# vkit-dev/vkit-ocr-model-adaptive-scaling

Measured on AMD Instinct MI355X. Metric: images/sec fwd+bwd @1024x1024 bf16 (train step: rough+precise passes, losses, backward, clip, AdamW), higher is better.
Workload: dtype bf16

## Files before the change

include/vkas.h:

```cpp
#ifndef VKAS_H
#define VKAS_H

#include <stddef.h>
#include <stdint.h>

#ifdef __cplusplus
extern "C" {
#endif

#define VKAS_F32 0
#define VKAS_BF16 1
#define VKAS_F16 2

#define VKAS_OK 0
#define VKAS_E_ARG (-1)
#define VKAS_E_LAUNCH (-2)

#define VKAS_EPI_NONE 0
#define VKAS_EPI_GELU 1
#define VKAS_EPI_SCALE_RES 2
#define VKAS_EPI_DGELU 3
#define VKAS_EPI_ADD 4
#define VKAS_EPI_PATCH 5
#define VKAS_EPI_HEAD 6
// ... 77 lines not shown
                       const float* colscale, const float* rowscale, int rows_per_image, void* h, long ldh, void* z,
                       long ldz, void* out, long ldo, long M, int C, int dtype, void* stream);
int vkas_mlp_chain_ln_fwd(const void* y, long ldy, const float* ln_gamma, const float* ln_beta, void* yn, long ldyn,
                          float* stats, const void* img, const float* b2, const void* x, long ldx, const float* colscale,
                          const float* rowscale, int rows_per_image, void* h, long ldh, void* z, long ldz, void* out,
                          long ldo, long M, int C, int dtype, void* stream);
int vkas_mlp_chain_bwd(const void* dz, long lddz, const void* img_t, const void* h, long ldh, void* dh, long lddh,
                       void* dyn, long lddyn, long M, int C, int dtype, void* stream);
int vkas_conv_gemm_tile(int wgrad, long M, int Np, int K);
int vkas_conv_gemm_kernel_id(int wgrad, const vkas_conv_geom* g, int Np, long lddy, int head_width);
typedef struct vkas_gemm_switches {
  int nt_tile, tn_tile;
  int nt_ring;
  int nt_noslab, nt_nobuf, tn_nobuf, tn_noslab, tn_no96;
} vkas_gemm_switches;
typedef struct vkas_gemm_plan_info {
  int kernel_id, family, bn, ring, buf, head, pw, nobias, xg;
  long grid_m, grid_n, tiles, splits, rows, a_bytes, b_bytes;
  unsigned grid;
  char name[44];
} vkas_gemm_plan_info;
int vkas_conv_gemm_plan(int wgrad, const vkas_conv_geom* g, int Np, long lddy, int head_width, int flags, int has_gb,
                        const vkas_gemm_switches* sw, vkas_gemm_plan_info* out);
int vkas_colsum(const void* y, long ld, long M, int Np, float* out, int accumulate, float* ws, size_t ws_bytes,
                int dtype, void* stream);
size_t vkas_colsum_ws_bytes(long M, int Np);

int vkas_dwconv7x7_fwd(const void* x, long ldx, const float* w, const float* bias, const void* addend, long ldadd,
                       void* y, long ldy, int B, int H, int W, int Cp, int dtype, void* stream);
int vkas_dwconv7x7_wgrad(const void* x, long ldx, const void* dy, long lddy, float* gw, float* gb, float* ws,
                         size_t ws_bytes, int B, int H, int W, int Cp, int dtype, void* stream);
size_t vkas_dwconv7x7_wgrad_ws_bytes(int B, int H, int W, int Cp);

int vkas_layernorm_fwd(const void* x, long ldx, const float* gamma, const float* beta, void* y, long ldy,
                       float* stats, long M, int C, int Cp, int act_gelu, int dtype, void* stream);
int vkas_layernorm_bwd(const void* x, long ldx, const float* gamma, const float* beta, const float* stats,
                       const void* dy, long lddy, void* dx, long lddx, float* dgamma, float* dbeta, float* ws,
                       size_t ws_bytes, long M, int C, int Cp, int act_gelu, int dtype, void* stream);
size_t vkas_layernorm_bwd_ws_bytes(long M, int Cp);

int vkas_pack_head_params(const float* gamma, const float* beta, const float* wproj, const float* bproj, int C, int oc,
                          int pw, float* out, void* stream);
int vkas_head_tail_fwd(const void* z, long ldz, const vkas_head_desc* hd, long M, int dtype, void* stream);
int vkas_head_tail_bwd(const void* z, long ldz, const vkas_head_desc* hd, const float* const* dproj, void* dz, long lddz,
                       float* dparams, float* ws, size_t ws_bytes, long M, int dtype, void* stream);
size_t vkas_head_tail_bwd_ws_bytes(long M, int pw);
// ... 165 lines not shown
```

vkit_ocr_model_adaptive_scaling_amd/_lib.py:

```python
import ctypes
import os
from ctypes import POINTER, Structure, c_char, c_char_p, c_double, c_float, c_int, c_int64, c_long, c_longlong, c_size_t, c_uint, c_void_p

_HERE = os.path.dirname(os.path.abspath(__file__))
LIB_PATH = os.environ.get('VKAS_LIB_PATH') or os.path.join(_HERE, 'libvkas.so')

F32, BF16, F16 = 0, 1, 2
EPI_NONE, EPI_GELU, EPI_SCALE_RES, EPI_DGELU, EPI_ADD, EPI_PATCH, EPI_HEAD = range(7)
LOSS_FOCAL, LOSS_DICE, LOSS_L1, LOSS_SMOOTH_L1, LOSS_L2 = range(5)
LOSS_WAHR = 5
PRECISE_LOSS_EX_SUMS = 16


class ConvGeom(Structure):
    _fields_ = [('B', c_int), ('Hin', c_int), ('Win', c_int), ('Hout', c_int), ('Wout', c_int), ('Cp', c_int),
                ('ldx', c_int), ('KH', c_int), ('KW', c_int), ('stride', c_int), ('pad', c_int)]


class HeadDesc(Structure):
    _fields_ = [('n_heads', c_int), ('pw', c_int), ('n0', c_int * 4), ('np', c_int * 4), ('c', c_int * 4),
                ('oc', c_int * 4), ('params', c_void_p), ('stats', c_void_p), ('proj', c_void_p)]


class Epilogue(Structure):
    _fields_ = [('mode', c_int), ('bias', c_void_p), ('out', c_void_p), ('ldo', c_long), ('out2', c_void_p),
                ('ldo2', c_long), ('aux', c_void_p), ('ldaux', c_long), ('colscale', c_void_p),
                ('rowscale', c_void_p), ('rows_per_image', c_int), ('patch', c_int), ('patch_Hs', c_int),
                ('patch_Ws', c_int), ('patch_Cp', c_int), ('head', HeadDesc)]


class GemmSwitches(Structure):
    _fields_ = [('nt_tile', c_int), ('tn_tile', c_int), ('nt_ring', c_int), ('nt_noslab', c_int), ('nt_nobuf', c_int),
                ('tn_nobuf', c_int), ('tn_noslab', c_int), ('tn_no96', c_int)]

    def __init__(self, nt_ring=-1, **kw):
        super().__init__(nt_ring=nt_ring, **kw)


class GemmPlanInfo(Structure):
    _fields_ = [(n, c_int) for n in ('kernel_id', 'family', 'bn', 'ring', 'buf', 'head', 'pw', 'nobias', 'xg')] + \
               [(n, c_long) for n in ('grid_m', 'grid_n', 'tiles', 'splits', 'rows', 'a_bytes', 'b_bytes')] + \
               [('grid', c_uint), ('name', c_char * 44)]


class PackDesc(Structure):
    _fields_ = [('w', c_void_p), ('out', c_void_p), ('total', c_long), ('kind', c_int), ('N', c_int), ('C', c_int),
                ('KH', c_int), ('KW', c_int), ('Np', c_int), ('Cp', c_int), ('mode', c_int), ('n_off', c_int),
                ('Nt', c_int), ('dtype', c_int)]


class RoughLossCfg(Structure):
    _fields_ = [('focal_factor', c_float), ('dice_factor', c_float), ('l1_factor', c_float), ('score_min', c_float),
                ('height_min', c_float), ('focal_alpha', c_float), ('focal_gamma', c_float), ('out_scale', c_float)]


class PreciseLossCfg(Structure):
    _fields_ = [('pos_l2', c_float), ('neg_l2', c_float), ('offset_l1', c_float), ('reg_l1', c_float),
                ('angle_ce', c_float), ('dist_l1', c_float), ('loss_factor', c_float), ('smooth_beta', c_float),
                ('out_scale', c_float)]


class PreciseLossExtraCfg(Structure):
    _fields_ = [('mask_focal', c_float), ('prob_l1', c_float), ('prob_wahr', c_float), ('prob_l1_beta', c_float),
                ('wahr_gamma', c_float), ('focal_alpha', c_float), ('focal_gamma', c_float)]

# ... 31 lines not shown
    'vkas_nchw_f32_to_nhwc': (c_int, [_P, _P, c_long, c_int, c_int, c_int, c_int, c_int, c_int, _P]),
    'vkas_conv_gemm_fwd': (c_int, [_P, POINTER(ConvGeom), _P, c_int, POINTER(Epilogue), c_int, _P]),
    'vkas_conv_gemm_wgrad': (c_int, [_P, POINTER(ConvGeom), _P, c_long, c_int, _P, _P, c_int, _P]),
    'vkas_conv_gemm_wgrad_ordered': (c_int, [_P, POINTER(ConvGeom), _P, c_long, c_int, _P, c_int, _P]),
    'vkas_conv_gemm_wgrad_gelu': (c_int, [_P, POINTER(ConvGeom), _P, c_long, c_int, _P, _P, c_int, _P]),
    'vkas_upconv5_fold_elems': (c_size_t, [c_int, c_int, c_int, c_int]),
    'vkas_upconv5_fold': (c_int, [_P, _P, c_int, c_int, c_int, c_int, c_int, c_int, c_int, _P]),
    'vkas_upconv5_fwd': (c_int, [_P, POINTER(ConvGeom), c_int, _P, c_int, _P, _P, c_long, c_int, _P]),
    'vkas_upconv5_dgrad': (c_int, [_P, c_long, POINTER(ConvGeom), c_int, _P, c_int, _P, c_long, c_int, _P]),
    'vkas_upconv5_wgrad_ws_bytes': (c_size_t, [c_int, c_int, c_int, c_int]),
    'vkas_upconv5_wgrad': (c_int, [_P, POINTER(ConvGeom), c_int, _P, c_long, c_int, _P, c_size_t, _P, _P, c_int, _P]),
    'vkas_upconv5_unfold_wgrad': (c_int, [_P, _P, c_int, c_int, c_int, c_int, c_int, c_int, _P]),
    'vkas_mlp_chain_image_elems': (c_size_t, [c_int]),
    'vkas_mlp_chain_pack': (c_int, [_P, _P, _P, c_int, c_int, _P, c_int, _P]),
    'vkas_mlp_chain_fwd': (c_int, [_P, c_long, _P, _P, _P, c_long, _P, _P, c_int, _P, c_long, _P, c_long, _P, c_long,
                                   c_long, c_int, c_int, _P]),
    'vkas_mlp_chain_ln_fwd': (c_int, [_P, c_long, _P, _P, _P, c_long, _P, _P, _P, _P, c_long, _P, _P, c_int, _P, c_long, _P,
                                      c_long, _P, c_long, c_long, c_int, c_int, _P]),
    'vkas_mlp_chain_bwd': (c_int, [_P, c_long, _P, _P, c_long, _P, c_long, _P, c_long, c_long, c_int, c_int, _P]),
    'vkas_conv_gemm_tile': (c_int, [c_int, c_long, c_int, c_int]),
    'vkas_conv_gemm_kernel_id': (c_int, [c_int, POINTER(ConvGeom), c_int, c_long, c_int]),
    'vkas_conv_gemm_plan': (c_int, [c_int, POINTER(ConvGeom), c_int, c_long, c_int, c_int, c_int, POINTER(GemmSwitches),
                                    POINTER(GemmPlanInfo)]),
    'vkas_colsum': (c_int, [_P, c_long, c_long, c_int, _P, c_int, _P, c_size_t, c_int, _P]),
    'vkas_colsum_ws_bytes': (c_size_t, [c_long, c_int]),
    'vkas_dwconv7x7_fwd': (c_int, [_P, c_long, _P, _P, _P, c_long, _P, c_long, c_int, c_int, c_int, c_int, c_int, _P]),
    'vkas_dwconv7x7_wgrad': (c_int, [_P, c_long, _P, c_long, _P, _P, _P, c_size_t, c_int, c_int, c_int, c_int, c_int, _P]),
    'vkas_dwconv7x7_wgrad_ws_bytes': (c_size_t, [c_int, c_int, c_int, c_int]),
    'vkas_layernorm_fwd': (c_int, [_P, c_long, _P, _P, _P, c_long, _P, c_long, c_int, c_int, c_int, c_int, _P]),
    'vkas_layernorm_bwd': (c_int, [_P, c_long, _P, _P, _P, _P, c_long, _P, c_long, _P, _P, _P, c_size_t, c_long, c_int,
                                   c_int, c_int, c_int, _P]),
    'vkas_layernorm_bwd_ws_bytes': (c_size_t, [c_long, c_int]),
    'vkas_pack_head_params': (c_int, [_P, _P, _P, _P, c_int, c_int, c_int, _P, _P]),
    'vkas_head_tail_fwd': (c_int, [_P, c_long, _P, c_long, c_int, _P]),
    'vkas_head_tail_bwd': (c_int, [_P, c_long, POINTER(HeadDesc), POINTER(c_void_p), _P, c_long, _P, _P, c_size_t, c_long, c_int, _P]),
    'vkas_head_tail_bwd_ws_bytes': (c_size_t, [c_long, c_int]),
    'vkas_scale_res_bwd': (c_int, [_P, c_long, _P, c_long, _P, _P, c_int, _P, c_long, _P, _P, _P, c_size_t, c_long,
                                   c_int, c_int, _P]),
    'vkas_scale_res_bwd_ws_bytes': (c_size_t, [c_long, c_int]),
    'vkas_resize_fwd': (c_int, [_P, c_long, _P, c_long, c_int, c_int, c_int, c_int, c_int, c_int, c_int, c_int, c_int, _P]),
    'vkas_resize_bwd': (c_int, [_P, c_long, _P, c_long, c_int, c_int, c_int, c_int, c_int, c_int, c_int, c_int, c_int, _P]),
    'vkas_resize_bwd_ws_bytes': (c_size_t, [c_int, c_int, c_int, c_int, c_int, c_int]),
    'vkas_resize_bwd_ws': (c_int, [_P, c_long, _P, c_long, _P, c_size_t, c_int, c_int, c_int, c_int, c_int, c_int, c_int, c_int,
                                   c_int, _P]),
    'vkas_upconv_adj': (c_int, [_P, c_long, _P, c_int, c_int, c_int, c_int, c_int, _P]),
    'vkas_upconv_adj_colsum_ws_bytes': (c_size_t, [c_int, c_int, c_int, c_int]),
# ... 67 lines not shown
```

vkit_ocr_model_adaptive_scaling_amd/csrc/gemm_api.hip:

```cpp
#include <stdlib.h>
#include <string.h>

#include "gemm_parts.h"
#include "gemm_plan.h"

int vkas_gemm_nt_simple(const void*, const vkas_conv_geom*, const void*, int, const vkas_epilogue*, int, hipStream_t);
int vkas_gemm_tn_simple(const void*, const vkas_conv_geom*, const void*, long, int, float*, float*, int, int, hipStream_t);
int vkas_gemm_nt_mfma_bf16(const void*, const vkas_conv_geom*, const void*, int, const vkas_epilogue*, hipStream_t);
int vkas_gemm_tn_mfma_bf16(const void*, const vkas_conv_geom*, const void*, long, int, float*, float*, int, hipStream_t);
int vkas_gemm_nt_mfma_f16(const void*, const vkas_conv_geom*, const void*, int, const vkas_epilogue*, hipStream_t);
int vkas_gemm_tn_mfma_f16(const void*, const vkas_conv_geom*, const void*, long, int, float*, float*, int, hipStream_t);

static thread_local char g_err[512] = "";

void vkas_set_error(const char* fmt, ...) {
  va_list ap;
  va_start(ap, fmt);
  vsnprintf(g_err, sizeof(g_err), fmt, ap);
  va_end(ap);
}

extern "C" const char* vkas_last_error(void) { return g_err; }
extern "C" int vkas_abi_version(void) { return 1; }

static bool force_simple() {
  static int v = -1;
  if (v < 0) {
// ... 71 lines not shown

extern "C" int vkas_conv_gemm_plan(int wgrad, const vkas_conv_geom* g, int Np, long lddy, int head_width, int flags, int has_gb,
                                   const vkas_gemm_switches* sw, vkas_gemm_plan_info* out) {
  VKAS_CHECK(g && out, "vkas_conv_gemm_plan: null argument");
  vkas_gemm_plan_info o = {};
  if (!sw && force_simple()) {
    snprintf(o.name, sizeof(o.name), wgrad ? "gemm_tn_simple" : "gemm_nt_simple");
  } else if (wgrad) {
    const vkas_tn_plan p = vkas_plan_tn(*g, Np, lddy, flags, has_gb != 0, sw ? *sw : *vkas_gemm_env_switches());
    o = {vkas_tn_kernel_id(p), p.family, p.tile, 0, p.buf, 0, p.pw, p.nobias, p.xg, 0, 0, p.tiles, p.splits, p.rows, p.x_bytes, p.dy_bytes, p.grid, ""};
    const char* t = p.tile == 128 ? "2,2,4" : (p.tile == 192 ? "2,4,6" : (p.tile == 224 ? "2,4,7" : "4,2,6"));
    if (p.family == VKAS_TN_SLAB) snprintf(o.name, sizeof(o.name), "conv3x3_wgrad_slab_kernel<%d>", p.tile / 16);
    else snprintf(o.name, sizeof(o.name), "gemm_tn_mfma_kernel<%s,4>", t);
  } else {
    const vkas_nt_plan p = vkas_plan_nt(*g, Np, head_width, sw ? *sw : *vkas_gemm_env_switches());
    const long tiles = p.grid_m * p.grid_n;
    o = {vkas_nt_kernel_id(p), p.family, p.bn, p.ring, p.buf, p.head, 0, 0, 0, p.grid_m, p.grid_n, tiles, 1, 0, p.a_bytes, p.b_bytes, (unsigned)tiles, ""};
    if (p.family == VKAS_NT_SLAB) snprintf(o.name, sizeof(o.name), "conv3x3_slab_mfma_kernel<%d,%d>", p.bn / 32, (int)p.head);
    else if (p.family == VKAS_NT_RING) snprintf(o.name, sizeof(o.name), "gemm_nt_ring_kernel<%d>", p.ring);
    else snprintf(o.name, sizeof(o.name), "gemm_nt_mfma_kernel<%s,4,%d>", p.family == VKAS_NT_REG128 ? "2,2" : "4,2", p.bn / 32);
  }
  *out = o;
  return VKAS_OK;
}

extern "C" int vkas_conv_gemm_tile(int wgrad, long M, int Np, int K) {
  if (force_simple()) return 0;
  const vkas_gemm_switches& sw = *vkas_gemm_env_switches();
  return wgrad ? vkas_tn_tile_rule(M, Np, K, sw) : vkas_nt_tile_rule(M, Np, sw);
}

extern "C" int vkas_conv_gemm_kernel_id(int wgrad, const vkas_conv_geom* g, int Np, long lddy, int head_width) {
  vkas_gemm_plan_info o;
  return g && vkas_conv_gemm_plan(wgrad, g, Np, lddy, head_width, 0, 0, nullptr, &o) == VKAS_OK ? o.kernel_id : 0;
}

static int conv_gemm_wgrad(const char* who, const void* x, const vkas_conv_geom* g, const void* dy, long lddy, int Np,
                           float* gw, float* gb, int x_gelu, int dtype, void* stream) {
  int rc = vkas_check_geom(who, x, g, Np);
  if (rc) return rc;
  VKAS_CHECK(dy && vkas_aligned16(dy) && lddy >= Np && lddy % 8 == 0, "%s: bad dy (lddy=%ld)", who, lddy);
  VKAS_CHECK(gw, "%s: null gw", who);
  if (dtype == VKAS_BF16 && !force_simple())
    return vkas_gemm_tn_mfma_bf16(x, g, dy, lddy, Np, gw, gb, x_gelu, vkas_stream(stream));
  if (dtype == VKAS_F16 && !force_simple())
    return vkas_gemm_tn_mfma_f16(x, g, dy, lddy, Np, gw, gb, x_gelu, vkas_stream(stream));
// ... 183 lines not shown
```

vkit_ocr_model_adaptive_scaling_amd/csrc/gemm_mfma.hip:

```cpp
#include <stdlib.h>

#include <type_traits>

#include "gemm_parts.h"
#include "gemm_plan.h"

#ifdef VKAS_MFMA_F16
typedef f16_t elem_t;
typedef f16x8 elem8;
typedef f16x4 elem4;
#define VKAS_MFMA16(a, b, c, x, y, z) __builtin_amdgcn_mfma_f32_16x16x32_f16(a, b, c, x, y, z)
#define VKAS_MFMA_FN(name) name##_f16
#else
typedef bf16_t elem_t;
typedef bf16x8 elem8;
typedef bf16x4 elem4;
#define VKAS_MFMA16(a, b, c, x, y, z) __builtin_amdgcn_mfma_f32_16x16x32_bf16(a, b, c, x, y, z)
#define VKAS_MFMA_FN(name) name##_bf16
#endif

namespace {

constexpr int BK = 64;

#ifndef VKAS_ABL
#define VKAS_ABL 0
#endif
constexpr int ABL = VKAS_ABL;
// ... 80 lines not shown
      load8(hp + (2 + qq) * pw + c0, w);
#pragma unroll
      for (int c = 0; c < 8; ++c) pr[qq] = fmaf(a[c], w[c], pr[qq]);
    }
  }
#pragma unroll
  for (int qq = 0; qq < 4; ++qq) {
    if (qq >= oc) break;
    pr[qq] = group_sum<LPR>(pr[qq]);
  }
  if (j == 0 && m < M) {
    const float4 bp = *reinterpret_cast<const float4*>(hp + 6 * pw);
    float* po = e.head.proj + ((long)head * M + m) * 8;
    *reinterpret_cast<float4*>(po) = make_float4(pr[0] + bp.x, pr[1] + bp.y, pr[2] + bp.z, pr[3] + bp.w);
    *reinterpret_cast<float4*>(po + 4) = make_float4(0.f, 0.f, 0.f, 0.f);
    if (e.head.stats) {
      float* st = e.head.stats + ((long)head * M + m) * 2;
      st[0] = mean;
      st[1] = rstd;
    }
  }
}

template <int WM, int WN, int TM, int TN, bool HEAD>
__device__ __forceinline__ void nt_epilogue(f32x4 (&acc)[TM][TN], float* stage, const vkas_epilogue& e, int tile_n,
                                            long m0, long M, int n0, int n_end, int tid) {
  constexpr int NTHR = WM * WN * 64;
  constexpr int BM = WM * TM * 16, BN = WN * TN * 16;
  constexpr int VPR = BN / 8;
  const int lane = tid & 63;
  const int wave = tid >> 6;
  const int wm = wave / WN, wn = wave % WN;
  if constexpr (!HEAD) {
    constexpr int PB = BN * 2 + 16;
    static_assert(BM * PB <= 2 * (BM + BN) * BK * 2, "single-pass staging must fit the tile buffers");
    char* st = reinterpret_cast<char*>(stage);
#pragma unroll
    for (int j = 0; j < TN; ++j) {
      const int cl = wn * TN * 16 + j * 16 + (lane >> 4) * 4;
      float4 b = make_float4(0.f, 0.f, 0.f, 0.f);
      if (e.bias && n0 + cl < n_end) b = *reinterpret_cast<const float4*>(e.bias + n0 + cl);
#pragma unroll
      for (int i = 0; i < TM; ++i) {
        const int row = wm * TM * 16 + i * 16 + (lane & 15);
        float v[4] = {acc[i][j][0] + b.x, acc[i][j][1] + b.y, acc[i][j][2] + b.z, acc[i][j][3] + b.w};
        store4(reinterpret_cast<elem_t*>(st + row * PB) + cl, v);
      }
    }
    constexpr int NIT = (BM * VPR + NTHR - 1) / NTHR;
    const bool pre = e.aux != nullptr && (e.mode == VKAS_EPI_SCALE_RES || e.mode == VKAS_EPI_DGELU || e.mode == VKAS_EPI_ADD);
    Raw8<elem_t> auxr[NIT];
    if (pre) {
#pragma unroll
      for (int it = 0; it < NIT; ++it) {
        const int t = tid + it * NTHR;
        const int row = t / VPR, c8 = t - row * VPR;
        const long m = m0 + row;
        const int n = n0 + c8 * 8;
        auxr[it].zero();
        if (t < BM * VPR && m < M && n < n_end) auxr[it].load(reinterpret_cast<const elem_t*>(e.aux) + m * e.ldaux + n);
      }
    }
    __syncthreads();
    vkas_epilogue e2 = e;
    e2.bias = nullptr;
    if (pre) {
#pragma unroll
      for (int it = 0; it < NIT; ++it) {
        const int t = tid + it * NTHR;
        const int row = t / VPR, c8 = t - row * VPR;
        const long m = m0 + row;
        const int n = n0 + c8 * 8;
        if (t < BM * VPR && m < M && n < n_end) {
          float v[8];
          load8(reinterpret_cast<const elem_t*>(st + row * PB) + c8 * 8, v);
          epi_store8<elem_t>(e2, m, n, v, &auxr[it]);
        }
      }
    } else {
#pragma unroll 2
      for (int t = tid; t < BM * VPR; t += NTHR) {
        const int row = t / VPR, c8 = t - row * VPR;
        const long m = m0 + row;
        const int n = n0 + c8 * 8;
        if (m < M && n < n_end) {
          float v[8];
          load8(reinterpret_cast<const elem_t*>(st + row * PB) + c8 * 8, v);
          epi_store8<elem_t>(e2, m, n, v);
        }
      }
    }
  } else {
    constexpr int EP = BN + 4;
    constexpr int ER = TM * 16;
    float* hp_s = stage + ER * EP;
    {
      const int pw = e.head.pw, PSZ = 6 * pw + 8;
      const float* src = e.head.params + (long)tile_n * PSZ;
      for (int i = tid; i < PSZ; i += NTHR) hp_s[i] = src[i];
    }
#pragma unroll 1
    for (int pass = 0; pass < WM; ++pass) {
      if (wm == pass) {
#pragma unroll
        for (int i = 0; i < TM; ++i)
#pragma unroll
          for (int j = 0; j < TN; ++j)
            *reinterpret_cast<f32x4*>(stage + (i * 16 + (lane & 15)) * EP + wn * TN * 16 + j * 16 + (lane >> 4) * 4) =
                acc[i][j];
      }
      __syncthreads();
      if constexpr ((ABL & 256) == 0)
        head_tail_rows<NTHR, ER, EP, VPR>(e, tile_n, stage, hp_s, m0 + (long)pass * ER, M, n0, n_end - n0, tid);
      __syncthreads();
    }
  }
}

template <int WM, int WN, int TM, int TN, bool BUF, bool HEAD>
__global__ __launch_bounds__(WM* WN * 64) void gemm_nt_mfma_kernel(const elem_t* __restrict__ x, vkas_conv_geom g,
                                                                  const elem_t* __restrict__ Bw, int Np, long M, int K,
                                                                  vkas_epilogue e, unsigned a_bytes, unsigned b_bytes) {
  constexpr int NTHR = WM * WN * 64;
  constexpr int BM = WM * TM * 16, BN = WN * TN * 16;
  constexpr int RSTEP = NTHR / 8;
  constexpr int ACH = BM / RSTEP;
  constexpr int BCH = (BN + RSTEP - 1) / RSTEP;
  static_assert(BM % RSTEP == 0, "A tile must be covered by whole staging passes");
  __shared__ __attribute__((aligned(16))) elem_t lds[2 * (BM + BN) * BK];
  const int tid = threadIdx.x;
  const int lane = tid & 63;
  const int wave = tid >> 6;
  const int wm = wave / WN, wn = wave % WN;
  constexpr bool head_mode = HEAD;
  const unsigned ntile_n = head_mode ? (unsigned)e.head.n_heads : (unsigned)((Np + BN - 1) / BN);
  VKAS_TR(0);
// ... 525 lines not shown
              acc[i][j] = VKAS_MFMA16(fb[h][j], fa[h][i], acc[i][j], 0, 0, 0);
        __builtin_amdgcn_s_setprio(0);
      }
      if (grp == 0) retire();
      if constexpr ((ABL & 4) == 0) __builtin_amdgcn_s_barrier();
      asm volatile("" ::: "memory");
    };
    sub(std::integral_constant<int, 0>{});
    sub(std::integral_constant<int, 1>{});
    sub(std::integral_constant<int, 2>{});
    ky = ky1;
    cb = cb1;
  };
  int s = 0;
  for (; s + 1 < NS; s += 2) {
    step(std::integral_constant<int, 0>{}, s);
    step(std::integral_constant<int, 1>{}, s + 1);
  }
  if (s < NS) step(std::integral_constant<int, 0>{}, s);
  if (grp == 0) __builtin_amdgcn_s_barrier();
  nt_epilogue<WM, WN, TM, TN, HEAD>(acc, (float*)lds, e, tile_n, m0, M, n0, n_end, tid);
}

template <int TN, bool HEAD>
__global__ __launch_bounds__(512) void conv3x3_slab_mfma_kernel(const elem_t* __restrict__ x, vkas_conv_geom g,
                                                                const elem_t* __restrict__ Bw, int Np, long M, int K,
                                                                vkas_epilogue e, unsigned a_bytes, unsigned b_bytes) {
  constexpr int BN = 32 * TN;
  __shared__ __attribute__((aligned(1024))) elem_t lds[2 * SLAB + 3 * BN * BK];
  const unsigned ntile_n = HEAD ? (unsigned)e.head.n_heads : (unsigned)((Np + BN - 1) / BN);
  const unsigned total = gridDim.x;
  const unsigned xcd = blockIdx.x & 7u, slot8 = blockIdx.x >> 3;
  const unsigned q8 = total >> 3, r8 = total & 7u;
  unsigned tile = (xcd < r8 ? xcd * (q8 + 1) : r8 * (q8 + 1) + (xcd - r8) * q8) + slot8;
  if constexpr (HEAD && (EXPS & 4) != 0) {
    if (ntile_n == 4 && (total & 31u) == 0) {
      const unsigned mt = total >> 2;
      const unsigned m_tile = (xcd & 3u) * (mt >> 2) + (slot8 >> 1);
      tile = m_tile * 4u + (xcd >> 2) * 2u + (slot8 & 1u);
    }
  }
  if constexpr (HEAD && TN == 7) {
    if (e.head.np[tile % ntile_n] <= 192) {
      conv3x3_slab_body<6, true, BN>(x, g, Bw, Np, M, K, e, a_bytes, b_bytes, (lds_elem*)lds, tile, ntile_n);
      return;
    }
  }
  conv3x3_slab_body<TN, HEAD, BN>(x, g, Bw, Np, M, K, e, a_bytes, b_bytes, (lds_elem*)lds, tile, ntile_n);
}

constexpr int TN_ROWS = VKAS_TN_ROWS;

__device__ __forceinline__ float dot2_ones(unsigned pair, float acc) {
#ifdef VKAS_MFMA_F16
  typedef _Float16 h2 __attribute__((ext_vector_type(2)));
  const h2 one = {(_Float16)1.0f, (_Float16)1.0f};
  return __builtin_amdgcn_fdot2(__builtin_bit_cast(h2, pair), one, acc, false);
#else
  typedef __bf16 b2 __attribute__((ext_vector_type(2)));
  const b2 one = {(__bf16)1.0f, (__bf16)1.0f};
  return __builtin_amdgcn_fdot2_f32_bf16(__builtin_bit_cast(b2, pair), one, acc, false);
#endif
}

template <int LD>
__device__ __forceinline__ elem8 tr_frag(const elem_t* tile, int mbase, int colbase, int lane) {
  const int g4 = lane >> 4, idx = lane & 15, q = idx >> 2, p = idx & 3;
  const elem_t* a0 = tile + (mbase + 4 * g4 + q) * LD + colbase + 4 * p;
  const elem_t* a1 = a0 + 16 * LD;
  const s16x4 lo = __builtin_amdgcn_ds_read_tr16_b64_v4i16((s16x4 __attribute__((address_space(3)))*)(a0));
  const s16x4 hi = __builtin_amdgcn_ds_read_tr16_b64_v4i16((s16x4 __attribute__((address_space(3)))*)(a1));
// ... 531 lines not shown
#if defined(VKAS_TRACE) && !defined(VKAS_MFMA_F16)
extern "C" int vkas_trace_read(void* dst, size_t bytes) {
  return (int)hipMemcpyFromSymbol(dst, HIP_SYMBOL(vkas_trace_buf), bytes, 0, hipMemcpyDeviceToHost);
}
#endif

static constexpr int nt_case(int family, int v, bool buf, bool head) { return ((family * 8 + v) * 2 + buf) * 2 + head; }
static constexpr int tn_case(int family, int tile, bool xg, int form) { return ((family * 512 + tile) * 2 + xg) * 4 + form; }

int VKAS_MFMA_FN(vkas_gemm_nt_mfma)(const void* x, const vkas_conv_geom* g, const void* Bw, int Np, const vkas_epilogue* e,
                           hipStream_t st) {
  const long M = (long)g->B * g->Hout * g->Wout;
  const int K = g->KH * g->KW * g->Cp;
  if (M == 0) return VKAS_OK;
  const bool head = e->mode == VKAS_EPI_HEAD;
  int wmax = 0;
  for (int h = 0; head && h < e->head.n_heads; ++h) wmax = e->head.np[h] > wmax ? e->head.np[h] : wmax;
  const vkas_nt_plan p = vkas_plan_nt(*g, Np, wmax, *vkas_gemm_env_switches());
  const dim3 grid((unsigned)(p.grid_m * (head ? e->head.n_heads : p.grid_n)));
  const unsigned ab = p.buf ? (unsigned)p.a_bytes : 0u, bb = p.buf ? (unsigned)p.b_bytes : 0u;
#define VKAS_GO(THREADS, ...) \
  __VA_ARGS__<<<grid, THREADS, 0, st>>>((const elem_t*)x, *g, (const elem_t*)Bw, Np, M, K, *e, ab, bb); \
  break;
#define VKAS_TILE(TNV)                                                                                      \
  case nt_case(VKAS_NT_TILE256, TNV, true, true): VKAS_GO(512, gemm_nt_mfma_kernel<4, 2, 4, TNV, true, true>)    \
  case nt_case(VKAS_NT_TILE256, TNV, false, true): VKAS_GO(512, gemm_nt_mfma_kernel<4, 2, 4, TNV, false, true>)  \
  case nt_case(VKAS_NT_TILE256, TNV, true, false): VKAS_GO(512, gemm_nt_mfma_kernel<4, 2, 4, TNV, true, false>)  \
  case nt_case(VKAS_NT_TILE256, TNV, false, false): VKAS_GO(512, gemm_nt_mfma_kernel<4, 2, 4, TNV, false, false>) \
  case nt_case(VKAS_NT_SLAB, TNV, true, true): VKAS_GO(512, conv3x3_slab_mfma_kernel<TNV, true>)                \
  case nt_case(VKAS_NT_SLAB, TNV, true, false): VKAS_GO(512, conv3x3_slab_mfma_kernel<TNV, false>)
  switch (nt_case(p.family, p.family == VKAS_NT_RING ? p.ring : p.bn / 32, p.buf, p.head)) {
    VKAS_TILE(4) VKAS_TILE(6) VKAS_TILE(7)
    case nt_case(VKAS_NT_REG128, 4, true, false): VKAS_GO(256, gemm_nt_mfma_kernel<2, 2, 4, 4, true, false>)
    case nt_case(VKAS_NT_REG128, 4, false, false): VKAS_GO(256, gemm_nt_mfma_kernel<2, 2, 4, 4, false, false>)
    case nt_case(VKAS_NT_RING, 2, true, false): VKAS_GO(512, gemm_nt_ring_kernel<2>)
    case nt_case(VKAS_NT_RING, 3, true, false): VKAS_GO(512, gemm_nt_ring_kernel<3>)
    case nt_case(VKAS_NT_RING, 4, true, false): VKAS_GO(512, gemm_nt_ring_kernel<4>)
    default: VKAS_CHECK(false, "gemm_nt_mfma: no kernel for family %d, N extent %d", (int)p.family, p.bn);
  }
#undef VKAS_TILE
#undef VKAS_GO
  static const char* const who[] = {"gemm_nt_mfma", "gemm_nt_ring", "gemm_nt_mfma", "conv3x3_slab_mfma"};
  VKAS_LAUNCH_CHECK(who[p.family]);
  return VKAS_OK;
}

int VKAS_MFMA_FN(vkas_gemm_tn_mfma)(const void* x, const vkas_conv_geom* g, const void* dy, long lddy, int Np, float* gw,
                           float* gb, int flags, hipStream_t st) {
  const long M = (long)g->B * g->Hout * g->Wout;
  const int K = g->KH * g->KW * g->Cp;
  if (M == 0) return VKAS_OK;
  const vkas_tn_plan p = vkas_plan_tn(*g, Np, lddy, flags, gb != nullptr, *vkas_gemm_env_switches());
  const unsigned xb = p.buf ? (unsigned)p.x_bytes : 0u, db = p.buf ? (unsigned)p.dy_bytes : 0u;
#define VKAS_GO(THREADS, ROWS, ...) \
  __VA_ARGS__<<<p.grid, THREADS, 0, st>>>((const elem_t*)x, *g, (const elem_t*)dy, lddy, Np, M, K, ROWS, gw, gb, xb, db); \
  break;
#define VKAS_TILE(WN, WK, TNn, XG)                                                                                             \
  case tn_case(VKAS_TN_GENERIC, WN * TNn * 16, XG, 0): VKAS_GO(WN * WK * 64, p.rows, gemm_tn_mfma_kernel<WN, WK, TNn, 4, false, XG>) \
  case tn_case(VKAS_TN_GENERIC, WN * TNn * 16, XG, 1): VKAS_GO(WN * WK * 64, p.rows, gemm_tn_mfma_kernel<WN, WK, TNn, 4, true, XG>)  \
  case tn_case(VKAS_TN_GENERIC, WN * TNn * 16, XG, 2): VKAS_GO(WN * WK * 64, p.rows, gemm_tn_mfma_kernel<WN, WK, TNn, 4, true, XG, true>)
  switch (tn_case(p.family, p.tile, p.xg, p.nobias ? 3 : (p.pw ? 2 : p.buf))) {
    VKAS_TILE(2, 2, 4, false) VKAS_TILE(2, 4, 6, false) VKAS_TILE(2, 4, 7, false) VKAS_TILE(4, 2, 6, false)
    VKAS_TILE(2, 2, 4, true) VKAS_TILE(2, 4, 6, true) VKAS_TILE(2, 4, 7, true) VKAS_TILE(4, 2, 6, true)
    case tn_case(VKAS_TN_GENERIC, 192, false, 3): VKAS_GO(512, p.rows, gemm_tn_mfma_kernel<2, 4, 6, 4, true, false, true, true>)
// ... 12 lines not shown
```

vkit_ocr_model_adaptive_scaling_amd/csrc/gemm_plan.h:

```cpp
#pragma once
#include "../../include/vkas.h"

constexpr int VKAS_TN_ROWS = 64;

enum vkas_nt_family { VKAS_NT_REG128, VKAS_NT_RING, VKAS_NT_TILE256, VKAS_NT_SLAB };
enum vkas_tn_family { VKAS_TN_GENERIC, VKAS_TN_SLAB };

struct vkas_nt_plan {
  vkas_nt_family family;
  int bn;
  int ring;
  bool buf, head;
  long a_bytes, b_bytes;
  long grid_m, grid_n;
};

struct vkas_tn_plan {
  vkas_tn_family family;
  int tile;
  bool buf, pw, nobias, xg;
  long splits, rows;
  long tiles;
  unsigned grid;
  long x_bytes, dy_bytes;
};

const vkas_gemm_switches* vkas_gemm_env_switches();

inline long vkas_span_bytes(long rows, long ld, long width) { return ((rows - 1) * ld + width) * 2; }
inline bool vkas_fits_buffer(long bytes) { return bytes < 0xFFFFFFF0L; }

int vkas_nt_tile_rule(long M, int Np, const vkas_gemm_switches& sw);
int vkas_tn_tile_rule(long M, int Np, int K, const vkas_gemm_switches& sw);

vkas_nt_plan vkas_plan_nt(const vkas_conv_geom& g, int Np, int head_width, const vkas_gemm_switches& sw);
vkas_tn_plan vkas_plan_tn(const vkas_conv_geom& g, int Np, long lddy, int flags, bool has_gb, const vkas_gemm_switches& sw);

inline int vkas_nt_kernel_id(const vkas_nt_plan& p) {
  return p.family == VKAS_NT_SLAB ? 1000 + p.bn / 32 : (p.family == VKAS_NT_RING ? 10 + p.ring : (p.family == VKAS_NT_REG128 ? 1 : p.bn));
}
inline int vkas_tn_kernel_id(const vkas_tn_plan& p) { return p.family == VKAS_TN_SLAB ? 2000 + p.tile / 16 : p.tile; }
```

vkit_ocr_model_adaptive_scaling_amd/csrc/gemm_plan.hip:

```cpp
#include "gemm_plan.h"

#include <stdlib.h>

#include <initializer_list>

static long cdiv(long a, long b) { return (a + b - 1) / b; }
static long padded(long n, long t) { return cdiv(n, t) * t; }

const vkas_gemm_switches* vkas_gemm_env_switches() {
  static const vkas_gemm_switches sw = [] {
    const auto num = [](const char* name, int unset) { return getenv(name) ? atoi(getenv(name)) : unset; };
    const auto set = [](const char* name) { return (int)(getenv(name) != nullptr); };
    return vkas_gemm_switches{num("VKAS_NT_TILE", 0), num("VKAS_TN_TILE", 0), num("VKAS_NT_RING", -1), set("VKAS_NT_NOSLAB"),
                              set("VKAS_NT_NOBUF"),   set("VKAS_TN_NOBUF"),   set("VKAS_TN_NOSLAB"),   set("VKAS_TN_NO96")};
  }();
  return &sw;
}

static bool row_aligned_3x3(const vkas_conv_geom& g, int wmod) {
  return g.KH == 3 && g.KW == 3 && g.stride == 1 && g.pad == 1 && g.Hout == g.Hin && g.Wout == g.Win && g.Win % wmod == 0;
}

int vkas_nt_tile_rule(long M, int Np, const vkas_gemm_switches& sw) {
  const int f = sw.nt_tile;
  if (f == 1 || f == 128 || f == 192 || f == 224) return f;
  if (M < 16384) return 1;
  int bn = 224;
  for (int c : {192, 128})
    if (padded(Np, c) < padded(Np, bn)) bn = c;
  return bn;
}

int vkas_tn_tile_rule(long M, int Np, int K, const vkas_gemm_switches& sw) {
  const int f = sw.tn_tile;
  if (f == 128 || f == 192 || f == 224 || f == 384) return f;
  int bn = 128;
  if (M >= 16384 && K >= 192) {
    for (int c : {192, 224})
      if (padded(Np, c) <= padded(Np, bn)) bn = c;
// ... 82 lines not shown
```

Before: 280.9.

## Add 2D band tiling form for 3x3 slab conv with row-piece slot ring

Adds a band variant of the 3x3 slab conv kernel in which each 256-row M tile covers a 4-row by 64-pixel image patch rather than a run of 256 pixels along one image row. Input rows are streamed as pieces into an 8-slot LDS ring and reused across the ky taps of neighbouring wave rows, with per-step waitcnt scheduling. The epilogue maps rows to the band layout. The form is on by default when the image height is divisible by 4, and it adds considerable complexity in the scheduling and in the vmcnt bookkeeping.

```diff
diff --git a/include/vkas.h b/include/vkas.h
--- a/include/vkas.h
+++ b/include/vkas.h
@@ -123,6 +123,14 @@
 } vkas_gemm_plan_info;
 int vkas_conv_gemm_plan(int wgrad, const vkas_conv_geom* g, int Np, long lddy, int head_width, int flags, int has_gb,
                         const vkas_gemm_switches* sw, vkas_gemm_plan_info* out);
+int vkas_conv_slab_form(int form);
+typedef struct vkas_slab_band_step {
+  int cb, ky, kx, fill_cb, fill_piece, fill_slot, read_slot[4], requests, wait;
+} vkas_slab_band_step;
+typedef struct vkas_slab_band_info {
+  int slots, slot_rows, slot_bytes, region_bytes, prologue_pieces, requests_per_piece;
+} vkas_slab_band_info;
+int vkas_conv_slab_band_schedule(int ncb, vkas_slab_band_info* info, vkas_slab_band_step* out, int cap);
 int vkas_colsum(const void* y, long ld, long M, int Np, float* out, int accumulate, float* ws, size_t ws_bytes,
                 int dtype, void* stream);
 size_t vkas_colsum_ws_bytes(long M, int Np);
diff --git a/vkit_ocr_model_adaptive_scaling_amd/_lib.py b/vkit_ocr_model_adaptive_scaling_amd/_lib.py
--- a/vkit_ocr_model_adaptive_scaling_amd/_lib.py
+++ b/vkit_ocr_model_adaptive_scaling_amd/_lib.py
@@ -41,6 +41,15 @@
     _fields_ = [(n, c_int) for n in ('kernel_id', 'family', 'bn', 'ring', 'buf', 'head', 'pw', 'nobias', 'xg')] + \
                [(n, c_long) for n in ('grid_m', 'grid_n', 'tiles', 'splits', 'rows', 'a_bytes', 'b_bytes')] + \
                [('grid', c_uint), ('name', c_char * 44)]
+
+
+class SlabBandStep(Structure):
+    _fields_ = [(n, c_int) for n in ('cb', 'ky', 'kx', 'fill_cb', 'fill_piece', 'fill_slot')] + \
+               [('read_slot', c_int * 4), ('requests', c_int), ('wait', c_int)]
+
+
+class SlabBandInfo(Structure):
+    _fields_ = [(n, c_int) for n in ('slots', 'slot_rows', 'slot_bytes', 'region_bytes', 'prologue_pieces', 'requests_per_piece')]
 
 
 class PackDesc(Structure):
@@ -118,6 +127,8 @@
     'vkas_conv_gemm_kernel_id': (c_int, [c_int, POINTER(ConvGeom), c_int, c_long, c_int]),
     'vkas_conv_gemm_plan': (c_int, [c_int, POINTER(ConvGeom), c_int, c_long, c_int, c_int, c_int, POINTER(GemmSwitches),
                                     POINTER(GemmPlanInfo)]),
+    'vkas_conv_slab_form': (c_int, [c_int]),
+    'vkas_conv_slab_band_schedule': (c_int, [c_int, POINTER(SlabBandInfo), POINTER(SlabBandStep), c_int]),
     'vkas_colsum': (c_int, [_P, c_long, c_long, c_int, _P, c_int, _P, c_size_t, c_int, _P]),
     'vkas_colsum_ws_bytes': (c_size_t, [c_long, c_int]),
     'vkas_dwconv7x7_fwd': (c_int, [_P, c_long, _P, _P, _P, c_long, _P, c_long, c_int, c_int, c_int, c_int, c_int, _P]),
diff --git a/vkit_ocr_model_adaptive_scaling_amd/csrc/gemm_api.hip b/vkit_ocr_model_adaptive_scaling_amd/csrc/gemm_api.hip
--- a/vkit_ocr_model_adaptive_scaling_amd/csrc/gemm_api.hip
+++ b/vkit_ocr_model_adaptive_scaling_amd/csrc/gemm_api.hip
@@ -3,6 +3,7 @@
 
 #include "gemm_parts.h"
 #include "gemm_plan.h"
+#include "slab_band_plan.h"
 
 int vkas_gemm_nt_simple(const void*, const vkas_conv_geom*, const void*, int, const vkas_epilogue*, int, hipStream_t);
 int vkas_gemm_tn_simple(const void*, const vkas_conv_geom*, const void*, long, int, float*, float*, int, int, hipStream_t);
@@ -120,6 +121,30 @@
   }
   *out = o;
   return VKAS_OK;
+}
+
+extern "C" int vkas_conv_slab_band_schedule(int ncb, vkas_slab_band_info* info, vkas_slab_band_step* out, int cap) {
+  if (ncb < 1 || cap < 0 || (cap > 0 && !out)) return -1;
+  if (info)
+    *info = {VKAS_BAND_SLOTS, VKAS_BAND_SLOT_ROWS, VKAS_BAND_SLOT_ROWS * 128, 2 * 264 * 128, VKAS_BAND_PROLOGUE, VKAS_BAND_REQ};
+  int n = 0, sb = 0;
+  for (int cb = 0; cb < ncb; ++cb, sb = vkas_band_slot(1, sb)) {
+    const bool nxt = cb + 1 < ncb;
+    for (int ky = 0; ky < 3; ++ky)
+      for (int kx = 0; kx < 3; ++kx, ++n) {
+        if (n >= cap) continue;
+        const bool more = ky < 2 || nxt;
+        const int piece = vkas_band_issue_piece(ky, kx);
+        vkas_slab_band_step s = {cb, ky, kx, -1, -1, -1, {0, 0, 0, 0}, 0, 0};
+        if (piece >= VKAS_BAND_PIECES && nxt) s.fill_cb = cb + 1, s.fill_piece = piece - VKAS_BAND_PIECES;
+        else if (piece >= 0 && piece < VKAS_BAND_PIECES) s.fill_cb = cb, s.fill_piece = piece;
+        if (s.fill_piece >= 0) s.fill_slot = (sb + piece) & (VKAS_BAND_SLOTS - 1), s.requests = VKAS_BAND_REQ;
+        for (int wm = 0; wm < 4; ++wm) s.read_slot[wm] = (sb + vkas_band_read_piece(ky, wm)) & (VKAS_BAND_SLOTS - 1);
+        s.wait = more ? vkas_band_requests(ky, kx, nxt) : -1;
+        out[n] = s;
+      }
+  }
+  return n;
 }
 
 extern "C" int vkas_conv_gemm_tile(int wgrad, long M, int Np, int K) {
diff --git a/vkit_ocr_model_adaptive_scaling_amd/csrc/gemm_mfma.hip b/vkit_ocr_model_adaptive_scaling_amd/csrc/gemm_mfma.hip
--- a/vkit_ocr_model_adaptive_scaling_amd/csrc/gemm_mfma.hip
+++ b/vkit_ocr_model_adaptive_scaling_amd/csrc/gemm_mfma.hip
@@ -4,6 +4,7 @@
 
 #include "gemm_parts.h"
 #include "gemm_plan.h"
+#include "slab_band_plan.h"
 
 #ifdef VKAS_MFMA_F16
 typedef f16_t elem_t;
@@ -130,9 +131,11 @@
   }
 }
 
-template <int WM, int WN, int TM, int TN, bool HEAD>
+template <int WM, int WN, int TM, int TN, bool HEAD, bool BAND = false>
 __device__ __forceinline__ void nt_epilogue(f32x4 (&acc)[TM][TN], float* stage, const vkas_epilogue& e, int tile_n,
-                                            long m0, long M, int n0, int n_end, int tid) {
+                                            long m0, long M, int n0, int n_end, int tid, int band_w = 0) {
+  static_assert(!BAND || TM * 16 == 64, "a wave row of the band form is one image row piece");
+  const auto mrow = [&](int row) -> long { return BAND ? m0 + (long)(row >> 6) * band_w + (row & 63) : m0 + row; };
   constexpr int NTHR = WM * WN * 64;
   constexpr int BM = WM * TM * 16, BN = WN * TN * 16;
   constexpr int VPR = BN / 8;
@@ -163,7 +166,7 @@
       for (int it = 0; it < NIT; ++it) {
         const int t = tid + it * NTHR;
         const int row = t / VPR, c8 = t - row * VPR;
-        const long m = m0 + row;
+        const long m = mrow(row);
         const int n = n0 + c8 * 8;
         auxr[it].zero();
         if (t < BM * VPR && m < M && n < n_end) auxr[it].load(reinterpret_cast<const elem_t*>(e.aux) + m * e.ldaux + n);
@@ -177,7 +180,7 @@
       for (int it = 0; it < NIT; ++it) {
         const int t = tid + it * NTHR;
         const int row = t / VPR, c8 = t - row * VPR;
-        const long m = m0 + row;
+        const long m = mrow(row);
         const int n = n0 + c8 * 8;
         if (t < BM * VPR && m < M && n < n_end) {
           float v[8];
@@ -189,7 +192,7 @@
 #pragma unroll 2
       for (int t = tid; t < BM * VPR; t += NTHR) {
         const int row = t / VPR, c8 = t - row * VPR;
-        const long m = m0 + row;
+        const long m = mrow(row);
         const int n = n0 + c8 * 8;
         if (m < M && n < n_end) {
           float v[8];
@@ -219,7 +222,7 @@
       }
       __syncthreads();
       if constexpr ((ABL & 256) == 0)
-        head_tail_rows<NTHR, ER, EP, VPR>(e, tile_n, stage, hp_s, m0 + (long)pass * ER, M, n0, n_end - n0, tid);
+        head_tail_rows<NTHR, ER, EP, VPR>(e, tile_n, stage, hp_s, mrow(pass * ER), M, n0, n_end - n0, tid);
       __syncthreads();
     }
   }
@@ -791,10 +794,194 @@
   nt_epilogue<WM, WN, TM, TN, HEAD>(acc, (float*)lds, e, tile_n, m0, M, n0, n_end, tid);
 }
 
+template <int TN, bool HEAD, int BNT>
+__device__ __forceinline__ void conv3x3_band_body(const elem_t* __restrict__ x, const vkas_conv_geom& g,
+                                                  const elem_t* __restrict__ Bw, int Np, long M, int K,
+                                                  const vkas_epilogue& e, unsigned a_bytes, unsigned b_bytes,
+                                                  lds_elem* lds, unsigned tile, unsigned ntile_n) {
+  constexpr int WM = 4, WN = 2, TM = 4;
+  constexpr int BN = WN * TN * 16;
+  constexpr int BT = BN * BK;
+  constexpr int NWI = BN / 8;
+  constexpr int NBQ = (NWI + 7) / 8;
+  constexpr int RAG = NWI % 8;
+  constexpr unsigned OOB = 0xFFFFFFF0u;
+  constexpr int PIX = VKAS_BAND_PIX;
+  constexpr int SLOT = VKAS_BAND_SLOT_ROWS * BK;
+  static_assert(VKAS_BAND_SLOTS * SLOT == 2 * SLAB, "the slot ring is the two slabs of the row form");
+  static_assert(WM == VKAS_BAND_ROWS && TM * 16 == PIX && VKAS_BAND_REQ == 2, "one wave row per image row, two requests per piece");
+  const int tid = threadIdx.x;
+  const int lane = tid & 63;
+  const int wave = __builtin_amdgcn_readfirstlane(tid >> 6);
+  const int wm = wave / WN, wn = wave % WN;
+  const int tile_n = (int)(tile % ntile_n);
+  const int n0 = HEAD ? e.head.n0[tile_n] : tile_n * BNT;
+  const int n_end = HEAD ? n0 + e.head.np[tile_n] : Np;
+  const int H = g.Hin, W = g.Win, Cp = g.Cp;
+  const unsigned mt = tile / ntile_n;
+  const unsigned nx = (unsigned)W / PIX, per_img = ((unsigned)H / VKAS_BAND_ROWS) * nx;
+  const int bimg = (int)(mt / per_img);
+  const unsigned rem = mt - (unsigned)bimg * per_img;
+  const int y0 = (int)(rem / nx) * VKAS_BAND_ROWS, x0 = (int)(rem % nx) * PIX;
+  const long m0 = ((long)bimg * H + y0) * W + x0;
+
+  const int lr = lane >> 3;
+  const int cl = (lane & 7) ^ lr;
+  const int cla = (lane & 7) ^ ((lr + 1) & 7);
+  const unsigned row_pitch = (unsigned)W * (unsigned)g.ldx * 2u;
+  const unsigned a_base = ((unsigned)((bimg * H + y0 - 1) * W + x0 + wave * 8 + lr) * (unsigned)g.ldx + (unsigned)(cla * 8)) * 2u;
+  const int hc = wave * 2 + (lane & 1);
+  const int hrow = hc >> 3;
+  const int hcl = (hc & 7) ^ hrow;
+  const int hpix = hrow == 0 ? x0 - 1 : x0 + PIX;
+  const bool h_ok = (unsigned)hpix < (unsigned)W;
+  const unsigned h_off = ((unsigned)((bimg * H + y0 - 1) * W + hpix) * (unsigned)g.ldx + (unsigned)(hcl * 8)) * 2u;
+  const int b_row = wave * 8 + lr;
+  const int b_rows = (n_end - n0 < BN) ? n_end - n0 : BN;
+  const unsigned b_base = ((unsigned)(n0 + b_row) * (unsigned)K + (unsigned)(cl * 8)) * 2u;
+  const unsigned b_qstep = 64u * (unsigned)K * 2u;
+  const __amdgpu_buffer_rsrc_t rs_a = __builtin_amdgcn_make_buffer_rsrc((void*)x, (short)0, (int)a_bytes, 0x00020000);
+  const __amdgpu_buffer_rsrc_t rs_b = __builtin_amdgcn_make_buffer_rsrc((void*)Bw, (short)0, (int)b_bytes, 0x00020000);
+  typedef __attribute__((address_space(3))) void* lds_ptr;
+
+  auto issue_a = [&](int p, int cb, int slot) {
+    const bool row_ok = (unsigned)(y0 - 1 + p) < (unsigned)H;
+    const unsigned step_off = (unsigned)p * row_pitch + (unsigned)cb * 128u;
+    lds_elem* dst = lds + slot * SLOT;
+    unsigned base = a_base;
+    asm volatile("" : "+v"(base));
+    const unsigned voff = (row_ok && cb * 64 + cla * 8 < Cp) ? base + step_off : OOB;
+    __builtin_amdgcn_raw_ptr_buffer_load_lds(rs_a, (lds_ptr)(dst + BK + wave * 512), 16, voff, 0, 0, 0);
+    unsigned hbase = h_off;
+    asm volatile("" : "+v"(hbase));
+    const unsigned hoff = (row_ok && h_ok && cb * 64 + hcl * 8 < Cp) ? hbase + step_off : OOB;
+    if (lane < 2)
+      __builtin_amdgcn_raw_ptr_buffer_load_lds(rs_a, (lds_ptr)(dst + (wave >> 2) * (PIX + 1) * BK + (wave & 3) * 16), 16, hoff, 0, 0, 0);
+  };
+  auto issue_b = [&](int ky, int kx, int cb, int slot) {
+    const unsigned step_off = ((unsigned)((ky * 3 + kx) * Cp) + (unsigned)cb * 64u) * 2u;
+    const bool c_ok = cb * 64 + cl * 8 < Cp;
+    lds_elem* dst = lds + 2 * SLAB + slot * BT;
+    unsigned base = b_base;
+    asm volatile("" : "+v"(base));
+#pragma unroll
+    for (int q = 0; q < NBQ; ++q) {
+      if (RAG != 0 && q == NBQ - 1 && wave >= RAG) break;
+      const unsigned voff = (c_ok && q * 64 + b_row < b_rows) ? base + (unsigned)q * b_qstep + step_off : OOB;
+      __builtin_amdgcn_raw_ptr_buffer_load_lds(rs_b, (lds_ptr)(dst + (q * 8 + wave) * 512), 16, voff, 0, 0, 0);
+    }
+  };
+
+  f32x4 acc[TM][TN];
+#pragma unroll
+  for (int j = 0; j < TN; ++j) {
+    f32x4 b4 = {0.f, 0.f, 0.f, 0.f};
+    if constexpr (HEAD) {
+      const int col = n0 + wn * TN * 16 + j * 16 + (lane >> 4) * 4;
+      if (e.bias && col < n_end) b4 = *reinterpret_cast<const f32x4*>(e.bias + col);
+    }
+#pragma unroll
+    for (int i = 0; i < TM; ++i) acc[i][j] = b4;
+  }
+
+  const int NCB = (Cp + 63) >> 6;
+#pragma unroll
+  for (int p = 0; p < VKAS_BAND_PROLOGUE; ++p) issue_a(p, 0, vkas_band_slot(0, p));
+  issue_b(0, 0, 0, 0);
+  issue_b(0, 1, 0, 1);
+  asm volatile("s_waitcnt vmcnt(0)" ::: "memory");
+  __builtin_amdgcn_s_barrier();
+  asm volatile("" ::: "memory");
+
+  const int frow = lane & 15, fchunk = lane >> 4;
+  unsigned fa_base[3];
+#pragma unroll
+  for (int kx = 0; kx < 3; ++kx) fa_base[kx] = (unsigned)swz_off(frow + kx, fchunk) * 2u;
+  const unsigned fb_base = (unsigned)swz_off(wn * TN * 16 + frow, fchunk) * 2u;
+  typedef const __attribute__((address_space(3))) char* lds_bytes;
+  const int grp = wave >> 2;
+  if (grp == 1) __builtin_amdgcn_s_barrier();
+  auto step = [&](auto kyc, int cb, int sb, bool nxt) {
+    constexpr int ky = decltype(kyc)::value;
+    const bool more = ky < 2 || nxt;
+    constexpr int ky1 = ky == 2 ? 0 : ky + 1;
+    const int cb1 = ky == 2 ? cb + 1 : cb;
+    const unsigned as_off = (unsigned)(((sb + vkas_band_read_piece(ky, wm)) & (VKAS_BAND_SLOTS - 1)) * SLOT * 2);
+    auto sub = [&](auto kxc) {
+      constexpr int kx = decltype(kxc)::value;
+      constexpr int PIECE = vkas_band_issue_piece(ky, kx);
+      auto retire = [&]() {
+        if (!more) {
+          asm volatile("s_waitcnt vmcnt(0)" ::: "memory");
+        } else if (PIECE < VKAS_BAND_PIECES || nxt) {
+          constexpr int NA = vkas_band_requests(ky, kx, true);
+          if (RAG != 0 && wave >= RAG) asm volatile("s_waitcnt vmcnt(%0)" ::"n"(NA + NBQ - (RAG != 0 ? 1 : 0)) : "memory");
+          else asm volatile("s_waitcnt vmcnt(%0)" ::"n"(NA + NBQ) : "memory");
+        } else {
+          constexpr int NA = vkas_band_requests(ky, kx, false);
+          if (RAG != 0 && wave >= RAG) asm volatile("s_waitcnt vmcnt(%0)" ::"n"(NA + NBQ - (RAG != 0 ? 1 : 0)) : "memory");
+          else asm volatile("s_waitcnt vmcnt(%0)" ::"n"(NA + NBQ) : "memory");
+        }
+      };
+      elem8 fa[2][TM], fb[2][TN];
+      const unsigned a0 = as_off + fa_base[kx];
+      const unsigned b0 = (unsigned)((2 * SLAB + kx * BT) * 2) + fb_base;
+#pragma unroll
+      for (int h = 0; h < 2; ++h) {
+#pragma unroll
+        for (int i = 0; i < TM; ++i)
+          fa[h][i] = *(const lds_elem8*)((lds_bytes)lds + ((a0 ^ (unsigned)(h * 64)) + (unsigned)(i * 16 * BK * 2)));
+#pragma unroll
+        for (int j = 0; j < TN; ++j)
+          fb[h][j] = *(const lds_elem8*)((lds_bytes)lds + ((b0 ^ (unsigned)(h * 64)) + (unsigned)(j * 16 * BK * 2)));
+      }
+      asm volatile("" ::: "memory");
+      if constexpr (PIECE >= VKAS_BAND_PIECES) {
+        if (nxt) issue_a(PIECE - VKAS_BAND_PIECES, cb + 1, (sb + PIECE) & (VKAS_BAND_SLOTS - 1));
+      } else if constexpr (PIECE >= 0) {
+        issue_a(PIECE, cb, (sb + PIECE) & (VKAS_BAND_SLOTS - 1));
+      }
+      if constexpr (kx == 0) issue_b(ky, 2, cb, 2);
+      else if (more) issue_b(ky1, kx - 1, cb1, kx - 1);
+      if (grp == 1) retire();
+      asm volatile("s_waitcnt lgkmcnt(0)" ::: "memory");
+      __builtin_amdgcn_s_barrier();
+      asm volatile("" ::: "memory");
+      __builtin_amdgcn_s_setprio(1);
+#pragma unroll
+      for (int h = 0; h < 2; ++h)
+#pragma unroll
+        for (int i = 0; i < TM; ++i)
+#pragma unroll
+          for (int j = 0; j < TN; ++j)
+            acc[i][j] = VKAS_MFMA16(fb[h][j], fa[h][i], acc[i][j], 0, 0, 0);
+      __builtin_amdgcn_s_setprio(0);
+      if (grp == 0) retire();
+      __builtin_amdgcn_s_barrier();
+      asm volatile("" ::: "memory");
+    };
+    sub(std::integral_constant<int, 0>{});
+    sub(std::integral_constant<int, 1>{});
+    sub(std::integral_constant<int, 2>{});
+  };
+  int sb = 0;
+#pragma unroll 1
+  for (int cb = 0; cb < NCB; ++cb) {
+    const bool nxt = cb + 1 < NCB;
+    step(std::integral_constant<int, 0>{}, cb, sb, nxt);
+    step(std::integral_constant<int, 1>{}, cb, sb, nxt);
+    step(std::integral_constant<int, 2>{}, cb, sb, nxt);
+    sb = vkas_band_slot(1, sb);
+  }
+  if (grp == 0) __builtin_amdgcn_s_barrier();
+  nt_epilogue<WM, WN, TM, TN, HEAD, true>(acc, (float*)lds, e, tile_n, m0, M, n0, n_end, tid, W);
+}
+
 template <int TN, bool HEAD>
 __global__ __launch_bounds__(512) void conv3x3_slab_mfma_kernel(const elem_t* __restrict__ x, vkas_conv_geom g,
                                                                 const elem_t* __restrict__ Bw, int Np, long M, int K,
-                                                                vkas_epilogue e, unsigned a_bytes, unsigned b_bytes) {
+                                                                vkas_epilogue e, unsigned a_bytes, unsigned b_bytes,
+                                                                int band) {
   constexpr int BN = 32 * TN;
   __shared__ __attribute__((aligned(1024))) elem_t lds[2 * SLAB + 3 * BN * BK];
   const unsigned ntile_n = HEAD ? (unsigned)e.head.n_heads : (unsigned)((Np + BN - 1) / BN);
@@ -811,11 +998,13 @@
   }
   if constexpr (HEAD && TN == 7) {
     if (e.head.np[tile % ntile_n] <= 192) {
-      conv3x3_slab_body<6, true, BN>(x, g, Bw, Np, M, K, e, a_bytes, b_bytes, (lds_elem*)lds, tile, ntile_n);
+      if (band) conv3x3_band_body<6, true, BN>(x, g, Bw, Np, M, K, e, a_bytes, b_bytes, (lds_elem*)lds, tile, ntile_n);
+      else conv3x3_slab_body<6, true, BN>(x, g, Bw, Np, M, K, e, a_bytes, b_bytes, (lds_elem*)lds, tile, ntile_n);
       return;
     }
   }
-  conv3x3_slab_body<TN, HEAD, BN>(x, g, Bw, Np, M, K, e, a_bytes, b_bytes, (lds_elem*)lds, tile, ntile_n);
+  if (band) conv3x3_band_body<TN, HEAD, BN>(x, g, Bw, Np, M, K, e, a_bytes, b_bytes, (lds_elem*)lds, tile, ntile_n);
+  else conv3x3_slab_body<TN, HEAD, BN>(x, g, Bw, Np, M, K, e, a_bytes, b_bytes, (lds_elem*)lds, tile, ntile_n);
 }
 
 constexpr int TN_ROWS = VKAS_TN_ROWS;
@@ -1393,13 +1582,17 @@
 #define VKAS_GO(THREADS, ...) \
   __VA_ARGS__<<<grid, THREADS, 0, st>>>((const elem_t*)x, *g, (const elem_t*)Bw, Np, M, K, *e, ab, bb); \
   break;
+  const int band = ABL == 0 && EXPS == 4 && vkas_slab_band_form() && g->Hin % VKAS_BAND_ROWS == 0;
+#define VKAS_GO_SLAB(...) \
+  __VA_ARGS__<<<grid, 512, 0, st>>>((const elem_t*)x, *g, (const elem_t*)Bw, Np, M, K, *e, ab, bb, band); \
+  break;
 #define VKAS_TILE(TNV)                                                                                      \
   case nt_case(VKAS_NT_TILE256, TNV, true, true): VKAS_GO(512, gemm_nt_mfma_kernel<4, 2, 4, TNV, true, true>)    \
   case nt_case(VKAS_NT_TILE256, TNV, false, true): VKAS_GO(512, gemm_nt_mfma_kernel<4, 2, 4, TNV, false, true>)  \
   case nt_case(VKAS_NT_TILE256, TNV, true, false): VKAS_GO(512, gemm_nt_mfma_kernel<4, 2, 4, TNV, true, false>)  \
   case nt_case(VKAS_NT_TILE256, TNV, false, false): VKAS_GO(512, gemm_nt_mfma_kernel<4, 2, 4, TNV, false, false>) \
-  case nt_case(VKAS_NT_SLAB, TNV, true, true): VKAS_GO(512, conv3x3_slab_mfma_kernel<TNV, true>)                \
-  case nt_case(VKAS_NT_SLAB, TNV, true, false): VKAS_GO(512, conv3x3_slab_mfma_kernel<TNV, false>)
+  case nt_case(VKAS_NT_SLAB, TNV, true, true): VKAS_GO_SLAB(conv3x3_slab_mfma_kernel<TNV, true>)                \
+  case nt_case(VKAS_NT_SLAB, TNV, true, false): VKAS_GO_SLAB(conv3x3_slab_mfma_kernel<TNV, false>)
   switch (nt_case(p.family, p.family == VKAS_NT_RING ? p.ring : p.bn / 32, p.buf, p.head)) {
     VKAS_TILE(4) VKAS_TILE(6) VKAS_TILE(7)
     case nt_case(VKAS_NT_REG128, 4, true, false): VKAS_GO(256, gemm_nt_mfma_kernel<2, 2, 4, 4, true, false>)
@@ -1411,6 +1604,7 @@
   }
 #undef VKAS_TILE
 #undef VKAS_GO
+#undef VKAS_GO_SLAB
   static const char* const who[] = {"gemm_nt_mfma", "gemm_nt_ring", "gemm_nt_mfma", "conv3x3_slab_mfma"};
   VKAS_LAUNCH_CHECK(who[p.family]);
   return VKAS_OK;
diff --git a/vkit_ocr_model_adaptive_scaling_amd/csrc/gemm_plan.h b/vkit_ocr_model_adaptive_scaling_amd/csrc/gemm_plan.h
--- a/vkit_ocr_model_adaptive_scaling_amd/csrc/gemm_plan.h
+++ b/vkit_ocr_model_adaptive_scaling_amd/csrc/gemm_plan.h
@@ -27,6 +27,8 @@
 
 const vkas_gemm_switches* vkas_gemm_env_switches();
 
+bool vkas_slab_band_form();
+
 inline long vkas_span_bytes(long rows, long ld, long width) { return ((rows - 1) * ld + width) * 2; }
 inline bool vkas_fits_buffer(long bytes) { return bytes < 0xFFFFFFF0L; }
 
diff --git a/vkit_ocr_model_adaptive_scaling_amd/csrc/gemm_plan.hip b/vkit_ocr_model_adaptive_scaling_amd/csrc/gemm_plan.hip
--- a/vkit_ocr_model_adaptive_scaling_amd/csrc/gemm_plan.hip
+++ b/vkit_ocr_model_adaptive_scaling_amd/csrc/gemm_plan.hip
@@ -1,6 +1,7 @@
 #include "gemm_plan.h"
 
 #include <stdlib.h>
+#include <string.h>
 
 #include <initializer_list>
 
@@ -15,6 +16,20 @@
                               set("VKAS_NT_NOBUF"),   set("VKAS_TN_NOBUF"),   set("VKAS_TN_NOSLAB"),   set("VKAS_TN_NO96")};
   }();
   return &sw;
+}
+
+static int g_slab_form = -1;
+static bool slab_form_default() {
+  static const bool bands = [] {
+    const char* s = getenv("VKAS_SLAB_FORM");
+    return !(s && (strcmp(s, "rows") == 0 || strcmp(s, "0") == 0));
+  }();
+  return bands;
+}
+bool vkas_slab_band_form() { return g_slab_form < 0 ? slab_form_default() : g_slab_form != 0; }
+extern "C" int vkas_conv_slab_form(int form) {
+  g_slab_form = form < 0 ? -1 : (form != 0);
+  return (int)vkas_slab_band_form();
 }
 
 static bool row_aligned_3x3(const vkas_conv_geom& g, int wmod) {
diff --git a/vkit_ocr_model_adaptive_scaling_amd/csrc/slab_band_plan.h b/vkit_ocr_model_adaptive_scaling_amd/csrc/slab_band_plan.h
--- /dev/null
+++ b/vkit_ocr_model_adaptive_scaling_amd/csrc/slab_band_plan.h
@@ -0,0 +1,20 @@
+#pragma once
+
+constexpr int VKAS_BAND_ROWS = 4;
+constexpr int VKAS_BAND_PIX = 64;
+constexpr int VKAS_BAND_SLOT_ROWS = 66;
+constexpr int VKAS_BAND_SLOTS = 8;
+constexpr int VKAS_BAND_PIECES = 6;
+constexpr int VKAS_BAND_PROLOGUE = 4;
+constexpr int VKAS_BAND_REQ = 2;
+
+constexpr int vkas_band_issue_piece(int ky, int kx) {
+  const int u = 3 * ky + kx;
+  return u == 0 ? 4 : (u == 1 ? 5 : (u == 2 ? 6 : (u == 3 ? 7 : (u == 4 ? 8 : (u == 6 ? 9 : -1)))));
+}
+constexpr int vkas_band_slot(int cb, int p) { return (VKAS_BAND_PIECES * cb + p) & (VKAS_BAND_SLOTS - 1); }
+constexpr int vkas_band_read_piece(int ky, int wm) { return ky + wm; }
+constexpr int vkas_band_requests(int ky, int kx, bool next_block) {
+  const int p = vkas_band_issue_piece(ky, kx);
+  return p < 0 || (p >= VKAS_BAND_PIECES && !next_block) ? 0 : VKAS_BAND_REQ;
+}
```

Result: no change. 282.3, median of 6 (+0.5%).
